# yanyan-li/PlanarSLAM

Hardware: AMD Instinct MI355X
Metric: RGB-D frames/sec (extract+match+pose-opt) @640x480; 1->8-GPU batch scaling (higher is better)
Workload: dtype u8/f64

## Files before the change

include/planar_abi.h:

```cpp
#ifndef PLANAR_ABI_H
#define PLANAR_ABI_H

#include <stdint.h>

#ifdef __cplusplus
extern "C" {
#endif

#define PLANAR_OK 0
#define PLANAR_EINVAL (-1)
#define PLANAR_ENOMEM (-2)
#define PLANAR_EDEVICE (-3)
#define PLANAR_ECAPACITY (-4)
#define PLANAR_ESTATE (-5)

typedef struct planar_ctx planar_ctx;

typedef struct planar_keypoint {
    float x, y;
    float size;
    float angle;
    float response;
    int32_t octave;
    int32_t class_id;
// ... 292 lines not shown
typedef struct planar_lsd planar_lsd;
int planar_lsd_create(planar_ctx* ctx, int width, int height, int max_batch, planar_lsd** out);
void planar_lsd_destroy(planar_lsd* lsd);
int planar_lsd_max_segments(void);
int planar_lsd_scaled_size(planar_lsd* lsd, int* w, int* h);
int planar_lsd_set_tie_order(planar_lsd* lsd, int tie_order);
int planar_lsd_set_top_only(planar_lsd* lsd, int enable);
int planar_lsd_extract(planar_lsd* lsd, const uint8_t* gray, int B, int pitch, int64_t frame_stride, int max_lines, planar_keyline* keylines,
                       uint8_t* ldesc, double* line_eq, int32_t* n_lines);
int planar_lsd_extract_dev(planar_lsd* lsd, const uint8_t* d_gray, int B, int pitch, int64_t frame_stride, int max_lines,
                           planar_keyline* d_keylines, uint8_t* d_ldesc, double* d_line_eq, int32_t* d_n_lines);
int planar_lsd_preprocess_dev(planar_lsd* lsd, const uint8_t* d_gray, int B, int pitch, int64_t frame_stride);
int planar_lsd_detect_dev(planar_lsd* lsd, int B, int max_lines, planar_keyline* d_keylines, uint8_t* d_ldesc, double* d_line_eq, int32_t* d_n_lines);
int planar_lsd_check(planar_lsd* lsd, int B);
int planar_lsd_read_stage(planar_lsd* lsd, int frame, int stage, void* out, int64_t out_bytes);
int planar_lsd_set_profiling(planar_lsd* lsd, int enable);
int planar_lsd_get_profile(planar_lsd* lsd, double* total_ms, int64_t* calls);
#ifdef PLANAR_TEST_HOOKS
int planar_debug_std_sort_desc(planar_ctx* ctx, float* keys, int32_t* perm, int n);
#endif

typedef struct planar_peac planar_peac;
int planar_peac_create(planar_ctx* ctx, int width, int height, int max_batch, planar_peac** out);
void planar_peac_destroy(planar_peac* peac);
int planar_peac_max_planes(void);
int planar_peac_segment(planar_peac* peac, const uint16_t* depth, int B, int pitch_px, int64_t frame_stride_px, float fx, float fy,
                        float cx, float cy, float depth_factor, int32_t* labels, double* planes, int32_t* n_planes);
int planar_peac_segment_dev(planar_peac* peac, const uint16_t* d_depth, int B, int pitch_px, int64_t frame_stride_px, float fx, float fy,
                            float cx, float cy, float depth_factor, int32_t* d_labels, double* d_planes, int32_t* d_n_planes);
int planar_peac_debug_layout(planar_peac* peac, int64_t* out );
int planar_peac_debug_read(planar_peac* peac, int frame, int64_t offset, int64_t bytes, void* out);
int planar_peac_check(planar_peac* peac, int B);
int planar_peac_set_variant(planar_peac* peac, int clustering, int wide_below);
int planar_peac_set_profiling(planar_peac* peac, int enable);
int planar_peac_get_profile(planar_peac* peac, double* total_ms, int64_t* calls);
int planar_peac_read_timing(planar_peac* peac, int B, int64_t* out);

typedef struct planar_comm planar_comm;
typedef struct planar_comm_id { char internal[128]; } planar_comm_id;
int planar_comm_unique_id(planar_comm_id* out);
int planar_comm_create(planar_ctx* ctx, const planar_comm_id* id, int nranks, int rank, planar_comm** out);
typedef int (*planar_allreduce_fn)(void* user, double* buf, size_t n, int op);
int planar_comm_create_hosted(planar_ctx* ctx, planar_allreduce_fn allreduce, void* user, int nranks, int rank, planar_comm** out);
void planar_comm_destroy(planar_comm* comm);

#define PLANAR_BA_MONO 0
#define PLANAR_BA_STEREO 1
#define PLANAR_BA_LINE 2
#define PLANAR_BA_PLANE 3
#define PLANAR_BA_VERTICAL 4
#define PLANAR_BA_PARALLEL 5

typedef struct planar_ba_problem {
    int32_t n_kf;
    const float* kf_Tcw;
    const uint8_t* kf_fixed;
    int32_t n_lm;
    const uint8_t* lm_type;
    const double* lm_init;
    int32_t n_edges;
    const int32_t* e_kf;
    const int32_t* e_lm;
    const uint8_t* e_type;
    const double* e_meas;
    const float* e_inv_sigma2;
} planar_ba_problem;
// ... 135 lines not shown
```

planarslam_amd/_lib.py:

```python
from __future__ import annotations

import ctypes as C
import os

import numpy as np

_HERE = os.path.dirname(os.path.abspath(__file__))
LIB_PATH = os.path.join(_HERE, "libplanar_hip.so")
if os.environ.get("PLANAR_HIP_LIB"):
    _ov = os.path.abspath(os.environ["PLANAR_HIP_LIB"])
    if os.path.dirname(_ov) != _HERE:
        raise ImportError(f"PLANAR_HIP_LIB={_ov}: a developer override must be a library inside {_HERE}")
    import warnings
    warnings.warn(f"planarslam_amd: loading the developer build {_ov} instead of libplanar_hip.so (PLANAR_HIP_LIB)")
    LIB_PATH = _ov

KP_DTYPE = np.dtype([("x", "<f4"), ("y", "<f4"), ("size", "<f4"), ("angle", "<f4"), ("response", "<f4"),
                     ("octave", "<i4"), ("class_id", "<i4")])


class PlanarError(RuntimeError):
    def __init__(self, code: int, msg: str):
        super().__init__(f"libplanar_hip error {code}: {msg}")
        self.code = code
# ... 134 lines not shown
    "planar_lsd_search_by_projection_dev": (C.c_int, [C.c_void_p, C.c_int, C.c_void_p, C.c_int, C.c_void_p, C.c_void_p, C.c_void_p, C.c_void_p, C.c_int] +
                                            [C.c_void_p] * 6 + [C.c_void_p, C.c_int, C.c_float, C.c_float, C.c_void_p, C.c_void_p]),
    "planar_plane_search_by_coefficients": (C.c_int, [C.c_void_p, C.c_int, C.c_void_p, C.c_int, C.c_void_p, C.c_void_p, C.c_int, C.c_void_p, C.c_int,
                                                      C.c_void_p, C.c_void_p, C.c_void_p, C.c_int, C.c_void_p, C.c_void_p] + [C.c_void_p] * 4),
    "planar_plane_search_by_coefficients_dev": (C.c_int, [C.c_void_p, C.c_int, C.c_void_p, C.c_int, C.c_void_p, C.c_void_p, C.c_int, C.c_void_p, C.c_int,
                                                          C.c_void_p, C.c_void_p, C.c_void_p, C.c_int, C.c_void_p, C.c_void_p] + [C.c_void_p] * 4),
    "planar_lsd_create": (C.c_int, [C.c_void_p, C.c_int, C.c_int, C.c_int, C.POINTER(C.c_void_p)]),
    "planar_lsd_destroy": (None, [C.c_void_p]),
    "planar_lsd_max_segments": (C.c_int, []),
    "planar_lsd_set_tie_order": (C.c_int, [C.c_void_p, C.c_int]),
    "planar_lsd_set_top_only": (C.c_int, [C.c_void_p, C.c_int]),
    "planar_undistort_keypoints": (C.c_int, [C.c_void_p, C.c_int, C.c_void_p, C.c_void_p, C.c_int] + [C.c_float] * 4 + [C.c_void_p, C.c_void_p]),
    "planar_undistort_keypoints_dev": (C.c_int, [C.c_void_p, C.c_int, C.c_void_p, C.c_void_p, C.c_int] + [C.c_float] * 4 + [C.c_void_p, C.c_void_p]),
    "planar_plane_clouds_sort_stats": (C.c_int, [C.c_void_p, C.c_int, C.c_void_p]),
    "planar_plane_clouds_set_profiling": (C.c_int, [C.c_void_p, C.c_int]),
    "planar_plane_clouds_get_profile": (C.c_int, [C.c_void_p, C.c_void_p, C.c_void_p]),
    "planar_lsd_set_profiling": (C.c_int, [C.c_void_p, C.c_int]),
    "planar_lsd_get_profile": (C.c_int, [C.c_void_p, C.c_void_p, C.c_void_p]),
    "planar_lsd_scaled_size": (C.c_int, [C.c_void_p, C.POINTER(C.c_int), C.POINTER(C.c_int)]),
    "planar_lsd_extract": (C.c_int, [C.c_void_p, C.c_void_p, C.c_int, C.c_int, C.c_int64, C.c_int, C.c_void_p, C.c_void_p, C.c_void_p, C.c_void_p]),
    "planar_lsd_extract_dev": (C.c_int, [C.c_void_p, C.c_void_p, C.c_int, C.c_int, C.c_int64, C.c_int, C.c_void_p, C.c_void_p, C.c_void_p, C.c_void_p]),
    "planar_lsd_preprocess_dev": (C.c_int, [C.c_void_p, C.c_void_p, C.c_int, C.c_int, C.c_int64]),
    "planar_lsd_detect_dev": (C.c_int, [C.c_void_p, C.c_int, C.c_int, C.c_void_p, C.c_void_p, C.c_void_p, C.c_void_p]),
    "planar_lsd_check": (C.c_int, [C.c_void_p, C.c_int]),
    "planar_lsd_read_stage": (C.c_int, [C.c_void_p, C.c_int, C.c_int, C.c_void_p, C.c_int64]),
    "planar_debug_std_sort_desc": (C.c_int, [C.c_void_p, C.c_void_p, C.c_void_p, C.c_int]),
    "planar_peac_create": (C.c_int, [C.c_void_p, C.c_int, C.c_int, C.c_int, C.POINTER(C.c_void_p)]),
    "planar_peac_destroy": (None, [C.c_void_p]),
    "planar_peac_max_planes": (C.c_int, []),
    "planar_peac_segment": (C.c_int, [C.c_void_p, C.c_void_p, C.c_int, C.c_int, C.c_int64, C.c_float, C.c_float, C.c_float, C.c_float, C.c_float, C.c_void_p, C.c_void_p, C.c_void_p]),
    "planar_peac_segment_dev": (C.c_int, [C.c_void_p, C.c_void_p, C.c_int, C.c_int, C.c_int64, C.c_float, C.c_float, C.c_float, C.c_float, C.c_float, C.c_void_p, C.c_void_p, C.c_void_p]),
    "planar_peac_check": (C.c_int, [C.c_void_p, C.c_int]),
    "planar_peac_set_variant": (C.c_int, [C.c_void_p, C.c_int, C.c_int]),
    "planar_track_manhattan_frame": (C.c_int, [C.c_void_p, C.c_int, C.c_void_p, C.c_void_p, C.c_void_p, C.c_int, C.c_void_p, C.c_void_p, C.c_int, C.c_void_p, C.c_void_p, C.c_void_p, C.c_void_p]),
    "planar_track_manhattan_frame_dev": (C.c_int, [C.c_void_p, C.c_int, C.c_void_p, C.c_void_p, C.c_void_p, C.c_int, C.c_void_p, C.c_void_p, C.c_int, C.c_void_p, C.c_void_p, C.c_void_p, C.c_void_p]),
    "planar_peac_read_timing": (C.c_int, [C.c_void_p, C.c_int, C.c_void_p]),
    "planar_reset_matches_dev": (C.c_int, [C.c_void_p, C.c_void_p, C.c_int64]),
    "planar_blocked_mask_dev": (C.c_int, [C.c_void_p, C.c_void_p, C.c_int64, C.c_void_p]),
    "planar_merge_matches_dev": (C.c_int, [C.c_void_p, C.c_void_p, C.c_void_p, C.c_int, C.c_int64, C.c_void_p]),
    "planar_manhattan_pose_dev": (C.c_int, [C.c_void_p, C.c_int, C.c_void_p, C.c_void_p, C.c_void_p, C.c_void_p]),
    "planar_keypoint_fields_dev": (C.c_int, [C.c_void_p, C.c_void_p, C.c_int64, C.c_void_p, C.c_void_p]),
    "planar_add_scalar_i32_dev": (C.c_int, [C.c_void_p, C.c_void_p, C.c_int64, C.c_int, C.c_void_p]),
    "planar_copy_rows_dev": (C.c_int, [C.c_void_p, C.c_void_p, C.c_int64, C.c_void_p, C.c_int64, C.c_int64, C.c_int64]),
    "planar_peac_debug_layout": (C.c_int, [C.c_void_p, C.c_void_p]),
    "planar_peac_debug_read": (C.c_int, [C.c_void_p, C.c_int, C.c_int64, C.c_int64, C.c_void_p]),
    "planar_comm_unique_id": (C.c_int, [C.c_void_p]),
    "planar_comm_create": (C.c_int, [C.c_void_p, C.c_void_p, C.c_int, C.c_int, C.POINTER(C.c_void_p)]),
    "planar_vocab_create": (C.c_int, [C.c_void_p, C.c_int, C.c_int, C.c_int, C.c_void_p, C.c_void_p, C.c_void_p, C.c_void_p, C.POINTER(C.c_void_p)]),
    "planar_vocab_destroy": (None, [C.c_void_p]),
    "planar_vocab_words": (C.c_int, [C.c_void_p]),
    "planar_bow_transform": (C.c_int, [C.c_void_p, C.c_void_p, C.c_void_p, C.c_int, C.c_int, C.c_int] + [C.c_void_p] * 6),
    "planar_bow_transform_dev": (C.c_int, [C.c_void_p, C.c_void_p, C.c_void_p, C.c_int, C.c_int, C.c_int] + [C.c_void_p] * 6),
    "planar_is_line_good": (C.c_int, [C.c_void_p, C.c_int, C.c_void_p, C.c_void_p, C.c_int, C.c_void_p, C.c_int, C.c_int, C.c_int, C.c_int64, C.c_float, C.c_float, C.c_float, C.c_float, C.c_float] + [C.c_void_p] * 8),
    "planar_is_line_good_dev": (C.c_int, [C.c_void_p, C.c_int, C.c_void_p, C.c_void_p, C.c_int, C.c_void_p, C.c_int, C.c_int, C.c_int, C.c_int64, C.c_float, C.c_float, C.c_float, C.c_float, C.c_float] + [C.c_void_p] * 8),
    "planar_normals_create": (C.c_int, [C.c_void_p, C.c_int, C.c_int, C.c_int, C.POINTER(C.c_void_p)]),
    "planar_normals_destroy": (None, [C.c_void_p]),
    "planar_normals_count": (C.c_int, [C.c_void_p]),
    "planar_normals_grid": (C.c_int, [C.c_void_p, C.POINTER(C.c_int), C.POINTER(C.c_int), C.POINTER(C.c_int), C.POINTER(C.c_int)]),
    "planar_normals_compute": (C.c_int, [C.c_void_p, C.c_void_p, C.c_int, C.c_int, C.c_int64, C.c_float, C.c_float, C.c_float, C.c_float, C.c_float, C.c_void_p, C.c_void_p]),
    "planar_normals_compute_dev": (C.c_int, [C.c_void_p, C.c_void_p, C.c_int, C.c_int, C.c_int64, C.c_float, C.c_float, C.c_float, C.c_float, C.c_float, C.c_void_p,
                                            C.c_void_p, C.c_int]),
    "planar_plane_clouds_create": (C.c_int, [C.c_void_p, C.c_int, C.c_int, C.c_int, C.c_int, C.POINTER(C.c_void_p)]),
    "planar_plane_clouds_destroy": (None, [C.c_void_p]),
    "planar_plane_clouds_set_timing": (C.c_int, [C.c_void_p, C.c_int]),
    "planar_plane_clouds_read_timing": (C.c_int, [C.c_void_p, C.c_int, C.c_void_p]),
    "planar_plane_clouds_stride": (C.c_int, [C.c_void_p, C.POINTER(C.c_int), C.POINTER(C.c_int)]),
# ... 100 lines not shown
```

planarslam_amd/csrc/common.h:

```cpp
#pragma once
#include <hip/hip_runtime.h>

#include <cstdarg>
#include <cstdint>
#include <cstdio>
#include <cstring>
#include <vector>

#include "../../include/planar_abi.h"

namespace planar {

void set_error(const char* fmt, ...);

#define PLANAR_HIP_CHECK(expr)                                                                        \
    do {                                                                                              \
        hipError_t _e = (expr);                                                                       \
        if (_e != hipSuccess) {                                                                       \
            ::planar::set_error("%s failed: %s (%s:%d)", #expr, hipGetErrorString(_e), __FILE__, __LINE__); \
            return (_e == hipErrorOutOfMemory) ? PLANAR_ENOMEM : PLANAR_EDEVICE;                      \
        }                                                                                             \
    } while (0)

#define PLANAR_REQUIRE(cond, code, msg)                  \
// ... 117 lines not shown
        for (int i = 0; i < slots; i++) total_ms[i] = 0;
        int64_t counted = 0;
        for (size_t c = 0; c < used; c++) {
            if (marked[c] != slots + 1) continue;
            for (int i = 0; i < slots; i++) {
                float ms = 0;
                PLANAR_HIP_CHECK(hipEventElapsedTime(&ms, ev[c * (slots + 1) + i], ev[c * (slots + 1) + i + 1]));
                total_ms[i] += ms;
            }
            counted++;
        }
        *calls = counted;
        reset();
        return PLANAR_OK;
    }
};

#ifdef __HIPCC__
__device__ __forceinline__ void xcd_frame_block(int per_frame, int B, int& frame, int& blk) {
    const int n = (int)blockIdx.x, group = 8 * per_frame, full = (B >> 3) * group;
    if (n < full) { const int g = n / group, r = n - g * group; frame = g * 8 + (r & 7); blk = r >> 3; }
    else { const int r = n - full; frame = (B & ~7) + r / per_frame; blk = r - (r / per_frame) * per_frame; }
}
#endif

}

struct planar_ctx {
    int device = 0;
    hipStream_t own_stream = nullptr;
    hipStream_t stream = nullptr;
    planar::DevBuf scratch;
    hipStream_t seq_stream = nullptr;
    hipEvent_t seq_fork = nullptr, seq_join = nullptr;
    hipStream_t seq_begin() {
        if (!seq_stream) return stream;
        hipError_t e = hipEventRecord(seq_fork, stream);
        if (e == hipSuccess) e = hipStreamWaitEvent(seq_stream, seq_fork, 0);
        if (e == hipSuccess) return seq_stream;
        planar::set_error("planar_ctx: the fork to the side stream failed (%s): launching on the context's stream", hipGetErrorString(e));
        return stream;
    }
    int seq_end(hipStream_t sq) {
        if (!seq_stream || sq != seq_stream) return PLANAR_OK;
        PLANAR_HIP_CHECK(hipEventRecord(seq_join, sq));
        PLANAR_HIP_CHECK(hipStreamWaitEvent(stream, seq_join, 0));
        return PLANAR_OK;
    }
    int ensure_scratch(size_t bytes) {
        if (scratch.bytes >= bytes) return PLANAR_OK;
        if (scratch.p) (void)hipStreamSynchronize(stream);
        return scratch.alloc(bytes);
    }
    void* host_scratch = nullptr;
    size_t host_scratch_bytes = 0;
    int ensure_host_scratch(size_t bytes) {
        if (host_scratch_bytes >= bytes) return PLANAR_OK;
        if (host_scratch) { (void)hipStreamSynchronize(stream); (void)hipHostFree(host_scratch); host_scratch = nullptr; host_scratch_bytes = 0; }
        const size_t want = planar::align_up(bytes + bytes / 4, (size_t)4096);
        hipError_t e = hipHostMalloc(&host_scratch, want, hipHostMallocDefault);
        if (e != hipSuccess) { (void)hipGetLastError(); host_scratch = nullptr; planar::set_error("hipHostMalloc(%zu) failed: %s", want, hipGetErrorString(e)); return PLANAR_EDEVICE; }
        host_scratch_bytes = want;
        return PLANAR_OK;
    }
};
```

planarslam_amd/csrc/ctx.hip:

```cpp
#include "common.h"

namespace planar {
static thread_local char g_err[512] = "";
void set_error(const char* fmt, ...) {
    va_list ap;
    va_start(ap, fmt);
    vsnprintf(g_err, sizeof(g_err), fmt, ap);
    va_end(ap);
}
}

extern "C" {

const char* planar_last_error(void) { return planar::g_err; }
int planar_abi_version(void) { return 200; }

int planar_ctx_create(planar_ctx** out, int device) {
    PLANAR_REQUIRE(out != nullptr, PLANAR_EINVAL, "out is null");
    *out = nullptr;
    int n = 0;
    PLANAR_HIP_CHECK(hipGetDeviceCount(&n));
    PLANAR_REQUIRE(device >= 0 && device < n, PLANAR_EDEVICE, "no such HIP device");
    PLANAR_HIP_CHECK(hipSetDevice(device));
    planar_ctx* c = new (std::nothrow) planar_ctx();
    PLANAR_REQUIRE(c != nullptr, PLANAR_ENOMEM, "host allocation failed");
    c->device = device;
    hipError_t e = hipStreamCreateWithFlags(&c->own_stream, hipStreamNonBlocking);
    if (e != hipSuccess) { delete c; planar::set_error("hipStreamCreate failed: %s", hipGetErrorString(e)); return PLANAR_EDEVICE; }
    c->stream = c->own_stream;
    *out = c;
    return PLANAR_OK;
}

void planar_ctx_destroy(planar_ctx* ctx) {
    if (!ctx) return;
    if (ctx->seq_fork) (void)hipEventDestroy(ctx->seq_fork);
    if (ctx->seq_join) (void)hipEventDestroy(ctx->seq_join);
    if (ctx->host_scratch) (void)hipHostFree(ctx->host_scratch);
    if (ctx->own_stream) (void)hipStreamDestroy(ctx->own_stream);
    delete ctx;
}

int planar_ctx_set_stream(planar_ctx* ctx, void* s) {
    PLANAR_REQUIRE(ctx != nullptr, PLANAR_EINVAL, "ctx is null");
    ctx->stream = s ? (hipStream_t)s : ctx->own_stream;
    return PLANAR_OK;
}

int planar_cu_stream_create(int device, const uint32_t* cu_mask, int n_words, void** out_stream) {
    PLANAR_REQUIRE(out_stream && cu_mask && n_words >= 1 && n_words <= 32, PLANAR_EINVAL, "bad argument");
    *out_stream = nullptr;
    bool any = false;
    for (int i = 0; i < n_words; i++) any = any || cu_mask[i] != 0u;
    PLANAR_REQUIRE(any, PLANAR_EINVAL, "empty CU mask");
    PLANAR_HIP_CHECK(hipSetDevice(device));
    hipStream_t s = nullptr;
    PLANAR_HIP_CHECK(hipExtStreamCreateWithCUMask(&s, (uint32_t)n_words, cu_mask));
    *out_stream = (void*)s;
    return PLANAR_OK;
}

void planar_cu_stream_destroy(void* stream) { if (stream) (void)hipStreamDestroy((hipStream_t)stream); }

int planar_ctx_set_seq_stream(planar_ctx* ctx, void* s) {
    PLANAR_REQUIRE(ctx != nullptr, PLANAR_EINVAL, "ctx is null");
    PLANAR_HIP_CHECK(hipSetDevice(ctx->device));
    if (s && !ctx->seq_fork) {
        PLANAR_HIP_CHECK(hipEventCreateWithFlags(&ctx->seq_fork, hipEventDisableTiming));
        PLANAR_HIP_CHECK(hipEventCreateWithFlags(&ctx->seq_join, hipEventDisableTiming));
    }
    ctx->seq_stream = (hipStream_t)s;
    return PLANAR_OK;
}

void* planar_ctx_get_stream(planar_ctx* ctx) { return ctx ? (void*)ctx->stream : nullptr; }

int planar_ctx_sync(planar_ctx* ctx) {
    PLANAR_REQUIRE(ctx != nullptr, PLANAR_EINVAL, "ctx is null");
    PLANAR_HIP_CHECK(hipStreamSynchronize(ctx->stream));
    return PLANAR_OK;
}

}
```

planarslam_amd/csrc/peac.hip:

```cpp
#include "common.h"

#include "peac_common.h"

namespace planar {
namespace peac {

constexpr int NT_REFINE = 256;
constexpr int NT_REFINE_WIDE = 1024;

struct Lds {
    float* h_key; u16* h_id; u16* pool; u16* nb_off; u16* nb_cnt; u16* dsp; u16* dss; u16* rid; unsigned* nouse; signed char* blk;
};

__device__ __forceinline__ int lds_find(u16* parent, int x) {
    int r = x, guard = 0;
    while (parent[r] != r && ++guard < 8192) r = parent[r];
    guard = 0;
    while (parent[x] != r && ++guard < 8192) { const int nx = parent[x]; parent[x] = (u16)r; x = nx; }
    return r;
}
template <int NT, int FJ>
__device__ __forceinline__ void refine_frame(const Layout& L, const Intr& K, const Consts& C, const uint16_t* __restrict__ depth, int pitch_px,
                                             int64_t frame_stride_px, uint8_t* __restrict__ ws, int32_t* __restrict__ labels,
                                             int64_t label_stride, double* __restrict__ planes, int32_t* __restrict__ n_planes,
                                             int32_t* __restrict__ status, long long* __restrict__ timing, const int frame) {
    const int tid = threadIdx.x, lane = tid & 63, wave = tid >> 6;
    uint8_t* F = ws + (size_t)frame * L.frame_bytes;
    double* g_stats = (double*)(F + L.off_stats);
    double* g_geo = (double*)(F + L.off_geo);
    int* g_N = (int*)(F + L.off_N);
    signed char* member = (signed char*)(F + L.off_member);
    float* distMap = (float*)(F + L.off_dist);
    unsigned* queue = (unsigned*)(F + L.off_queue);
// ... 718 lines not shown
                                                  int64_t frame_stride_px, uint8_t* __restrict__ ws, int32_t* __restrict__ labels,
                                                  int64_t label_stride, double* __restrict__ planes, int32_t* __restrict__ n_planes,
                                                  int32_t* __restrict__ status, long long* __restrict__ timing) {
    refine_frame<NT_REFINE_WIDE, 4>(L, K, C, depth, pitch_px, frame_stride_px, ws, labels, label_stride, planes, n_planes, status, timing, (int)blockIdx.x);
}

__global__ void peac_order(const long long* __restrict__ timing, int B, int* __restrict__ order) {
    const int i = blockIdx.x * blockDim.x + threadIdx.x;
    if (i >= B) return;
    const long long ci = timing[(size_t)i * TSLOTS + 3];
    int rank = 0;
    for (int j = 0; j < B; j++) {
        const long long cj = timing[(size_t)j * TSLOTS + 3];
        rank += (cj > ci || (cj == ci && j < i)) ? 1 : 0;
    }
    order[rank] = i;
}

}
}

#include "peac_ahc2.h"

using namespace planar;

struct planar_peac {
    planar_ctx* ctx = nullptr;
    int W = 0, H = 0, max_batch = 0;
    peac::Layout L{};
    peac::Consts C{};
    int smem2 = 0, smem3 = 0, smem_refine = 0;
    int wide_below = 64;
    bool exact_only = false;
    DevBuf d_ws, d_status, d_timing, d_next, d_order;
    int order_B = 0;
    DevBuf d_depth, d_labels, d_planes, d_nplanes;
    LaunchProfile prof{4};
};

extern "C" {

int planar_peac_create(planar_ctx* ctx, int width, int height, int max_batch, planar_peac** out) {
    PLANAR_REQUIRE(ctx && out, PLANAR_EINVAL, "null argument");
    *out = nullptr;
    PLANAR_REQUIRE(width >= 2 * peac::WIN && height >= 2 * peac::WIN && width <= 4096 && height <= 4096, PLANAR_EINVAL, "image size out of range");
    PLANAR_REQUIRE(max_batch >= 1, PLANAR_EINVAL, "max_batch must be >= 1");
    PLANAR_HIP_CHECK(hipSetDevice(ctx->device));
    planar_peac* o = new (std::nothrow) planar_peac();
    PLANAR_REQUIRE(o != nullptr, PLANAR_ENOMEM, "host allocation failed");
    o->ctx = ctx; o->W = width; o->H = height; o->max_batch = max_batch;
    o->L = peac::make_layout(width, height);
    o->C = peac::make_consts();
    const peac::Layout& L = o->L;
    o->smem2 = peac::ahc2_smem_bytes(L);
    o->smem3 = peac::ahc3_smem_bytes(L);
    o->smem_refine = (int)((L.NB + 15) / 16 * 16);
    if (L.pool_cap > 65535 || L.NB2 > 65535 || o->smem2 > 160 * 1024 - 2048 || o->smem3 > o->smem2) {
        delete o;
        set_error("planar_peac_create: %dx%d = %d blocks of 10x10 pixels: the clustering kernel's LDS-resident queue holds about 10 900 (1280x720 fits, 1920x1080 does not)", width, height, L.NB);
        return PLANAR_EINVAL;
    }
    if (o->smem2 > 48 * 1024) {
        hipError_t e = hipSuccess;
        if (o->smem3 > 48 * 1024) e = hipFuncSetAttribute((const void*)peac::peac_ahc3, hipFuncAttributeMaxDynamicSharedMemorySize, o->smem3);
        if (e == hipSuccess) e = hipFuncSetAttribute((const void*)peac::peac_ahc2, hipFuncAttributeMaxDynamicSharedMemorySize, o->smem2);
        if (e != hipSuccess) { (void)hipGetLastError(); delete o; set_error("planar_peac_create: %d bytes of LDS per workgroup are not available: %s", o->smem2, hipGetErrorString(e)); return PLANAR_EINVAL; }
    }
    int rc;
    if ((rc = o->d_ws.alloc((size_t)max_batch * L.frame_bytes)) || (rc = o->d_status.alloc((size_t)max_batch * 4)) ||
        (rc = o->d_timing.alloc((size_t)max_batch * peac::TSLOTS * 8)) || (rc = o->d_next.alloc(256)) || (rc = o->d_order.alloc((size_t)max_batch * 4))) { delete o; return rc; }
    *out = o;
    return PLANAR_OK;
}

void planar_peac_destroy(planar_peac* p) { delete p; }
int planar_peac_set_variant(planar_peac* p, int clustering, int wide_below) {
    PLANAR_REQUIRE(p && clustering >= 0 && clustering <= 1, PLANAR_EINVAL, "bad argument");
    p->exact_only = clustering == 1;
    if (wide_below >= 0) p->wide_below = wide_below;
    return PLANAR_OK;
}
int planar_peac_max_planes(void) { return peac::MAX_PLANES; }

int planar_peac_segment_dev(planar_peac* p, const uint16_t* d_depth, int B, int pitch_px, int64_t frame_stride_px, float fx, float fy,
                            float cx, float cy, float depth_factor, int32_t* d_labels, double* d_planes, int32_t* d_n_planes) {
    PLANAR_REQUIRE(p && d_depth && d_labels && d_planes && d_n_planes, PLANAR_EINVAL, "null argument");
    PLANAR_REQUIRE(B >= 1 && B <= p->max_batch, PLANAR_EINVAL, "B must be in [1, max_batch]");
    PLANAR_REQUIRE(pitch_px >= p->W && frame_stride_px >= (int64_t)pitch_px * p->H, PLANAR_EINVAL, "pitch/frame_stride too small");
    hipStream_t st = p->ctx->stream;
    const peac::Intr K{fx, fy, cx, cy, depth_factor};
    int rc = p->prof.begin();
    if (rc) return rc;
    auto mark = [&]() { p->prof.mark(st); };
    PLANAR_HIP_CHECK(hipMemsetAsync(p->d_next.p, 0, 4, st));
    mark();
    hipLaunchKernelGGL(peac::peac_blocks, dim3((p->L.NB + 63) / 64, B), dim3(64), 0, st, p->L, K, d_depth, pitch_px, frame_stride_px, p->d_ws.as<uint8_t>());
    mark();
    {
        hipStream_t sq = p->ctx->seq_begin();
        if (!p->exact_only) {
            hipLaunchKernelGGL(peac::peac_ahc3, dim3(B), dim3(64), p->smem3, sq, p->L, p->C, p->d_ws.as<uint8_t>(), p->d_status.as<int32_t>(),
                               p->d_timing.as<long long>(), p->d_next.as<int>(), p->order_B == B ? p->d_order.as<int>() : nullptr, 0);
            hipLaunchKernelGGL(peac::peac_ahc2, dim3(B), dim3(64), p->smem2, sq, p->L, p->C, p->d_ws.as<uint8_t>(), p->d_status.as<int32_t>(),
                               p->d_timing.as<long long>(), p->d_next.as<int>(), nullptr, 1);
        } else
            hipLaunchKernelGGL(peac::peac_ahc2, dim3(B), dim3(64), p->smem2, sq, p->L, p->C, p->d_ws.as<uint8_t>(), p->d_status.as<int32_t>(),
                               p->d_timing.as<long long>(), p->d_next.as<int>(), p->order_B == B ? p->d_order.as<int>() : nullptr, 0);
        if ((rc = p->ctx->seq_end(sq))) return rc;
    }
    mark();
    hipLaunchKernelGGL(peac::peac_order, dim3((B + 255) / 256), dim3(256), 0, st, p->d_timing.as<long long>(), B, p->d_order.as<int>());
    mark();
    if (B <= p->wide_below)
        hipLaunchKernelGGL(peac::peac_refine_wide, dim3(B), dim3(peac::NT_REFINE_WIDE), p->smem_refine, st, p->L, K, p->C, d_depth, pitch_px, frame_stride_px,
                           p->d_ws.as<uint8_t>(), d_labels, (int64_t)p->W * p->H, d_planes, d_n_planes, p->d_status.as<int32_t>(), p->d_timing.as<long long>());
    else
        hipLaunchKernelGGL(peac::peac_refine, dim3(B), dim3(peac::NT_REFINE), p->smem_refine, st, p->L, K, p->C, d_depth, pitch_px, frame_stride_px,
                           p->d_ws.as<uint8_t>(), d_labels, (int64_t)p->W * p->H, d_planes, d_n_planes, p->d_status.as<int32_t>(), p->d_timing.as<long long>());
    mark();
    p->order_B = B;
    PLANAR_HIP_CHECK(hipGetLastError());
    return PLANAR_OK;
}

int planar_peac_set_profiling(planar_peac* p, int enable) {
    PLANAR_REQUIRE(p != nullptr, PLANAR_EINVAL, "peac is null");
    PLANAR_HIP_CHECK(hipStreamSynchronize(p->ctx->stream));
    p->prof.on = enable != 0;
    p->prof.reset();
    return PLANAR_OK;
}
int planar_peac_get_profile(planar_peac* p, double* total_ms , int64_t* calls) {
    PLANAR_REQUIRE(p && total_ms && calls, PLANAR_EINVAL, "null argument");
    PLANAR_HIP_CHECK(hipStreamSynchronize(p->ctx->stream));
    return p->prof.sum(total_ms, calls);
}

int planar_peac_read_timing(planar_peac* p, int B, int64_t* out) {
    PLANAR_REQUIRE(p && out && B >= 1 && B <= p->max_batch, PLANAR_EINVAL, "bad argument");
    PLANAR_HIP_CHECK(hipStreamSynchronize(p->ctx->stream));
    PLANAR_HIP_CHECK(hipMemcpy(out, p->d_timing.p, (size_t)B * peac::TSLOTS * 8, hipMemcpyDeviceToHost));
    return PLANAR_OK;
}

// ... 53 lines not shown
```

planarslam_amd/csrc/peac_ahc2.h:

```cpp
#pragma once
#include "peac_common.h"
#include "wave_ops.h"

namespace planar {
namespace peac {

constexpr unsigned TOMB = 0xFFFFu;
#define WFENCE() do { __builtin_amdgcn_fence(__ATOMIC_SEQ_CST, "wavefront"); __builtin_amdgcn_wave_barrier(); } while (0)
#define GFENCE() __threadfence_block()

__device__ __forceinline__ void stats_compute_u(const double s[9], int N, Geo& g) {
    const double sc = 1.0 / N;
    g.center[0] = s[0] * sc; g.center[1] = s[1] * sc; g.center[2] = s[2] * sc;
    const double k00 = s[3] - s[0] * s[0] * sc, k01 = s[6] - s[0] * s[1] * sc, k02 = s[8] - s[0] * s[2] * sc;
    const double k11 = s[4] - s[1] * s[1] * sc, k12 = s[7] - s[1] * s[2] * sc, k22 = s[5] - s[2] * s[2] * sc;
    double ev[3], v[3];
    eig33u(k00, k01, k11, k02, k12, k22, ev, v);
    const bool keep = v[0] * g.center[0] + v[1] * g.center[1] + v[2] * g.center[2] <= 0;
    g.normal[0] = keep ? v[0] : -v[0]; g.normal[1] = keep ? v[1] : -v[1]; g.normal[2] = keep ? v[2] : -v[2];
    g.mse = ev[0] * sc;
}

__host__ __device__ static inline size_t al8(size_t v) { return (v + 7) & ~(size_t)7; }
static inline int ahc2_smem_bytes(const Layout& L) {
// ... 928 lines not shown
    WFENCE();
    mark();
    {
        unsigned* o_nouse = (unsigned*)(F + L.off_h_nouse); unsigned* o_cval = (unsigned*)(F + L.off_h_cval);
        const int W32o = (NB2 + 31) / 32;
        for (int b0 = 0; b0 < NB2; b0 += 64) {
            const int id = b0 + lane;
            bool dead;
            if constexpr (FAST) {
                if (id < NB) dead = mp[id] != id || (rec(id)[2] >> 16) != (unsigned)id;
                else dead = id < n_nodes;
            } else dead = id < NB2 && mp[id] != id;
            const u64 dm = __ballot(dead);
            if (lane == 0) { o_nouse[b0 >> 5] = (unsigned)dm; if ((b0 >> 5) + 1 < W32o) o_nouse[(b0 >> 5) + 1] = (unsigned)(dm >> 32); }
        }
        if constexpr (FAST) {
            GFENCE();
            for (int id = lane; id < NB; id += 64) {
                const unsigned c = rec(id)[2] >> 16;
                if (mp[id] == id && c >= (unsigned)NB) atomicAnd(&o_nouse[c >> 5], ~(1u << (c & 31)));
            }
        }
        for (int t = lane; t < (NB2 + 31) / 32; t += 64) o_cval[t] = 0;
        for (int t = lane; t < MAX_PLANES; t += 64) g_hand[4 + t] = t < n_ext ? (FAST ? (int)(rec(s_ext[t])[2] >> 16) : s_ext[t]) : 0;
        if (lane == 0) {
            g_hand[0] = n_ext; g_hand[1] = err; g_hand[2] = n_nodes;
            status[frame] = err;
            if (timing) {
                for (int t = 0; t < 4; t++) timing[(size_t)frame * TSLOTS + t] = t < nph ? tphase[t] - tphase[0] : 0;
                timing[(size_t)frame * TSLOTS + 9] = n_nodes;
                timing[(size_t)frame * TSLOTS + 7] = ((long long)dbg_phases << 40) | ((long long)dbg_nodes << 20) | dbg_hits;
                timing[(size_t)frame * TSLOTS + 10] = dbg_big;
                timing[(size_t)frame * TSLOTS + 11] = dbg_bigsolves;
                for (int t = 0; t < 24; t++) timing[(size_t)frame * TSLOTS + 16 + t] = cyc[t];
            }
        }
    }
    return wave_uni(err);
}

__global__ __launch_bounds__(64, 2) void peac_ahc3(Layout L, Consts C, uint8_t* __restrict__ ws, int32_t* __restrict__ status,
                                                   long long* __restrict__ timing, int* __restrict__ next_frame, const int* __restrict__ order, int retry_inline) {
    __shared__ int s_frame;
    __shared__ AhcShared s_sh;
#if defined(PLANAR_AHC_PRIO) && !defined(PLANAR_WAVE_EMUL)
    __builtin_amdgcn_s_setprio(PLANAR_AHC_PRIO);
#endif
    if (threadIdx.x == 0) { const int k = atomicAdd(next_frame, 1); s_frame = order ? order[k] : k; }
    __syncthreads();
    const int st = ahc_frame<true>(L, C, ws, status, timing, s_frame, s_sh);
    if (st == ST_RETRY && retry_inline) {
        __syncthreads();
        ahc_frame<false>(L, C, ws, status, timing, s_frame, s_sh);
        if (timing && threadIdx.x == 0) timing[(size_t)s_frame * TSLOTS + 12] = 1;
    }
}
__global__ __launch_bounds__(64) void peac_ahc2(Layout L, Consts C, uint8_t* __restrict__ ws, int32_t* __restrict__ status,
                                                long long* __restrict__ timing, int* __restrict__ next_frame, const int* __restrict__ order, int only_retry) {
    __shared__ int s_frame;
    __shared__ AhcShared s_sh;
    if (threadIdx.x == 0) {
        if (only_retry) s_frame = status[blockIdx.x] == ST_RETRY ? (int)blockIdx.x : -1;
        else { const int k = atomicAdd(next_frame, 1); s_frame = order ? order[k] : k; }
    }
    __syncthreads();
    if (s_frame < 0) return;
    ahc_frame<false>(L, C, ws, status, timing, s_frame, s_sh);
}

}
}
```

planarslam_amd/planes.py:

```python
from __future__ import annotations

import ctypes as C

import numpy as np

from ._lib import Context, PlanarError, check, lib


class PlaneDetection:
    def __init__(self, width: int = 640, height: int = 480, max_batch: int = 1, ctx: Context | None = None):
        self.L = lib()
        self.ctx = ctx or Context(0)
        self.width, self.height, self.max_batch = width, height, max_batch
        h = C.c_void_p()
        check(self.L.planar_peac_create(self.ctx.h, width, height, max_batch, C.byref(h)))
        self.h = h
        self.max_planes = self.L.planar_peac_max_planes()

    def close(self):
        if getattr(self, "h", None):
            self.L.planar_peac_destroy(self.h)
            self.h = None

    def __del__(self):
        try:
            self.close()
        except Exception:
            pass

    def run(self, depth: np.ndarray, K=(535.4, 539.2, 320.1, 247.6), depth_factor: float = 1.0 / 5000.0):
        if depth.dtype != np.uint16:
            raise TypeError("depth image must be CV_16U (uint16)")
        single = depth.ndim == 2
        d = np.ascontiguousarray(depth[None] if single else depth)
        B, H, W = d.shape
        if (W, H) != (self.width, self.height):
            raise ValueError(f"detector was created for {self.width}x{self.height}, got {W}x{H}")
        labels = np.zeros((B, H, W), np.int32)
        planes = np.zeros((B, self.max_planes, 8), np.float64)
        n = np.zeros(B, np.int32)
        check(self.L.planar_peac_segment(self.h, d.ctypes.data, B, W, W * H, K[0], K[1], K[2], K[3], np.float32(depth_factor),
                                         labels.ctypes.data, planes.ctypes.data, n.ctypes.data))
        res = [(planes[b, :n[b]].copy(), labels[b]) for b in range(B)]
        return res[0] if single else res

    def segment_dev(self, d_depth, d_labels, d_planes, d_n, B, K=(535.4, 539.2, 320.1, 247.6), depth_factor=1.0 / 5000.0):
        check(self.L.planar_peac_segment_dev(self.h, d_depth, B, self.width, self.width * self.height, K[0], K[1], K[2], K[3],
                                             np.float32(depth_factor), d_labels, d_planes, d_n))


class SurfaceNormals:

    def __init__(self, width: int = 640, height: int = 480, max_batch: int = 1, ctx: Context | None = None):
        self.L = lib()
        self.ctx = ctx or Context(0)
        self.width, self.height, self.max_batch = width, height, max_batch
        h = C.c_void_p()
        check(self.L.planar_normals_create(self.ctx.h, width, height, max_batch, C.byref(h)))
        self.h = h
        self.count = check(self.L.planar_normals_count(self.h))

# ... 171 lines not shown
```

Before: 12670.

## Make PEAC clustering kernels persistent and size grids by occupancy and CU mask

The ahc3 and ahc2 clustering kernels become persistent loops. Each workgroup keeps pulling frames from an atomic counter, and the grid is sized from occupancy times the CU count, using the seq stream's CU mask when one is set. Frames that need a retry go onto a device-side list, so the retry pass runs a small fixed grid over only those frames instead of launching B workgroups that mostly exit. The order kernel moves onto the seq stream, and a cap on workgroups is exposed. This is meant to cut launch and scheduling overhead and to balance frames of uneven cost, at the price of more atomics and kernarg reloads inside the loop.

```diff
diff --git a/include/planar_abi.h b/include/planar_abi.h
--- a/include/planar_abi.h
+++ b/include/planar_abi.h
@@ -348,6 +348,7 @@
 int planar_peac_debug_read(planar_peac* peac, int frame, int64_t offset, int64_t bytes, void* out);
 int planar_peac_check(planar_peac* peac, int B);
 int planar_peac_set_variant(planar_peac* peac, int clustering, int wide_below);
+int planar_peac_set_max_workgroups(planar_peac* peac, int n);
 int planar_peac_set_profiling(planar_peac* peac, int enable);
 int planar_peac_get_profile(planar_peac* peac, double* total_ms, int64_t* calls);
 int planar_peac_read_timing(planar_peac* peac, int B, int64_t* out);
diff --git a/planarslam_amd/_lib.py b/planarslam_amd/_lib.py
--- a/planarslam_amd/_lib.py
+++ b/planarslam_amd/_lib.py
@@ -190,6 +190,7 @@
     "planar_peac_segment_dev": (C.c_int, [C.c_void_p, C.c_void_p, C.c_int, C.c_int, C.c_int64, C.c_float, C.c_float, C.c_float, C.c_float, C.c_float, C.c_void_p, C.c_void_p, C.c_void_p]),
     "planar_peac_check": (C.c_int, [C.c_void_p, C.c_int]),
     "planar_peac_set_variant": (C.c_int, [C.c_void_p, C.c_int, C.c_int]),
+    "planar_peac_set_max_workgroups": (C.c_int, [C.c_void_p, C.c_int]),
     "planar_track_manhattan_frame": (C.c_int, [C.c_void_p, C.c_int, C.c_void_p, C.c_void_p, C.c_void_p, C.c_int, C.c_void_p, C.c_void_p, C.c_int, C.c_void_p, C.c_void_p, C.c_void_p, C.c_void_p]),
     "planar_track_manhattan_frame_dev": (C.c_int, [C.c_void_p, C.c_int, C.c_void_p, C.c_void_p, C.c_void_p, C.c_int, C.c_void_p, C.c_void_p, C.c_int, C.c_void_p, C.c_void_p, C.c_void_p, C.c_void_p]),
     "planar_peac_read_timing": (C.c_int, [C.c_void_p, C.c_int, C.c_void_p]),
diff --git a/planarslam_amd/csrc/common.h b/planarslam_amd/csrc/common.h
--- a/planarslam_amd/csrc/common.h
+++ b/planarslam_amd/csrc/common.h
@@ -173,6 +173,7 @@
     hipStream_t stream = nullptr;
     planar::DevBuf scratch;
     hipStream_t seq_stream = nullptr;
+    int seq_cus = 0;
     hipEvent_t seq_fork = nullptr, seq_join = nullptr;
     hipStream_t seq_begin() {
         if (!seq_stream) return stream;
diff --git a/planarslam_amd/csrc/ctx.hip b/planarslam_amd/csrc/ctx.hip
--- a/planarslam_amd/csrc/ctx.hip
+++ b/planarslam_amd/csrc/ctx.hip
@@ -13,7 +13,7 @@
 extern "C" {
 
 const char* planar_last_error(void) { return planar::g_err; }
-int planar_abi_version(void) { return 200; }
+int planar_abi_version(void) { return 201; }
 
 int planar_ctx_create(planar_ctx** out, int device) {
     PLANAR_REQUIRE(out != nullptr, PLANAR_EINVAL, "out is null");
@@ -70,6 +70,12 @@
         PLANAR_HIP_CHECK(hipEventCreateWithFlags(&ctx->seq_join, hipEventDisableTiming));
     }
     ctx->seq_stream = (hipStream_t)s;
+    ctx->seq_cus = 0;
+    if (s) {
+        uint32_t mask[32] = {0};
+        if (hipExtStreamGetCUMask((hipStream_t)s, 32, mask) == hipSuccess) { for (uint32_t w : mask) ctx->seq_cus += __builtin_popcount(w); }
+        else (void)hipGetLastError();
+    }
     return PLANAR_OK;
 }
 
diff --git a/planarslam_amd/csrc/peac.hip b/planarslam_amd/csrc/peac.hip
--- a/planarslam_amd/csrc/peac.hip
+++ b/planarslam_amd/csrc/peac.hip
@@ -1,4 +1,6 @@
 #include "common.h"
+
+#include <algorithm>
 
 #include "peac_common.h"
 
@@ -783,6 +785,7 @@
     int smem2 = 0, smem3 = 0, smem_refine = 0;
     int wide_below = 64;
     bool exact_only = false;
+    int occ3 = 0, occ2 = 0, dev_cus = 0, max_wg = 0;
     DevBuf d_ws, d_status, d_timing, d_next, d_order;
     int order_B = 0;
     DevBuf d_depth, d_labels, d_planes, d_nplanes;
@@ -817,9 +820,19 @@
         if (e == hipSuccess) e = hipFuncSetAttribute((const void*)peac::peac_ahc2, hipFuncAttributeMaxDynamicSharedMemorySize, o->smem2);
         if (e != hipSuccess) { (void)hipGetLastError(); delete o; set_error("planar_peac_create: %d bytes of LDS per workgroup are not available: %s", o->smem2, hipGetErrorString(e)); return PLANAR_EINVAL; }
     }
+    {
+        hipError_t e = hipOccupancyMaxActiveBlocksPerMultiprocessor(&o->occ3, (const void*)peac::peac_ahc3, 64, (size_t)o->smem3);
+        if (e == hipSuccess) e = hipOccupancyMaxActiveBlocksPerMultiprocessor(&o->occ2, (const void*)peac::peac_ahc2, 64, (size_t)o->smem2);
+        if (e == hipSuccess) e = hipDeviceGetAttribute(&o->dev_cus, hipDeviceAttributeMultiprocessorCount, ctx->device);
+        if (e != hipSuccess || o->occ3 < 1 || o->occ2 < 1 || o->dev_cus < 1) {
+            (void)hipGetLastError(); delete o;
+            set_error("planar_peac_create: the clustering kernels' residency is not available: %s", hipGetErrorString(e));
+            return PLANAR_EDEVICE;
+        }
+    }
     int rc;
     if ((rc = o->d_ws.alloc((size_t)max_batch * L.frame_bytes)) || (rc = o->d_status.alloc((size_t)max_batch * 4)) ||
-        (rc = o->d_timing.alloc((size_t)max_batch * peac::TSLOTS * 8)) || (rc = o->d_next.alloc(256)) || (rc = o->d_order.alloc((size_t)max_batch * 4))) { delete o; return rc; }
+        (rc = o->d_timing.alloc((size_t)max_batch * peac::TSLOTS * 8)) || (rc = o->d_next.alloc(256 + (size_t)max_batch * 4)) || (rc = o->d_order.alloc((size_t)max_batch * 4))) { delete o; return rc; }
     *out = o;
     return PLANAR_OK;
 }
@@ -829,6 +842,11 @@
     PLANAR_REQUIRE(p && clustering >= 0 && clustering <= 1, PLANAR_EINVAL, "bad argument");
     p->exact_only = clustering == 1;
     if (wide_below >= 0) p->wide_below = wide_below;
+    return PLANAR_OK;
+}
+int planar_peac_set_max_workgroups(planar_peac* p, int n) {
+    PLANAR_REQUIRE(p && n >= 0, PLANAR_EINVAL, "bad argument");
+    p->max_wg = n;
     return PLANAR_OK;
 }
 int planar_peac_max_planes(void) { return peac::MAX_PLANES; }
@@ -843,24 +861,29 @@
     int rc = p->prof.begin();
     if (rc) return rc;
     auto mark = [&]() { p->prof.mark(st); };
-    PLANAR_HIP_CHECK(hipMemsetAsync(p->d_next.p, 0, 4, st));
+    PLANAR_HIP_CHECK(hipMemsetAsync(p->d_next.p, 0, (1 + peac::RETRY_LIST) * 4, st));
     mark();
     hipLaunchKernelGGL(peac::peac_blocks, dim3((p->L.NB + 63) / 64, B), dim3(64), 0, st, p->L, K, d_depth, pitch_px, frame_stride_px, p->d_ws.as<uint8_t>());
     mark();
     {
         hipStream_t sq = p->ctx->seq_begin();
+        const int cus = (sq != st && sq == p->ctx->seq_stream && p->ctx->seq_cus > 0) ? std::min(p->ctx->seq_cus, p->dev_cus) : p->dev_cus;
+        auto grid = [&](int per_cu) { const int g = std::min(B, per_cu * cus); return dim3((unsigned)(p->max_wg > 0 ? std::min(g, p->max_wg) : g)); };
+        int* d_next = p->d_next.as<int>();
+        const int* order = p->order_B == B ? p->d_order.as<int>() : nullptr;
         if (!p->exact_only) {
-            hipLaunchKernelGGL(peac::peac_ahc3, dim3(B), dim3(64), p->smem3, sq, p->L, p->C, p->d_ws.as<uint8_t>(), p->d_status.as<int32_t>(),
-                               p->d_timing.as<long long>(), p->d_next.as<int>(), p->order_B == B ? p->d_order.as<int>() : nullptr, 0);
-            hipLaunchKernelGGL(peac::peac_ahc2, dim3(B), dim3(64), p->smem2, sq, p->L, p->C, p->d_ws.as<uint8_t>(), p->d_status.as<int32_t>(),
-                               p->d_timing.as<long long>(), p->d_next.as<int>(), nullptr, 1);
+            hipLaunchKernelGGL(peac::peac_ahc3, grid(p->occ3), dim3(64), p->smem3, sq, p->L, p->C, p->d_ws.as<uint8_t>(), p->d_status.as<int32_t>(),
+                               p->d_timing.as<long long>(), d_next, order, 0, B, d_next + 1);
+            const int g2 = std::min(B, peac::RETRY_GRID);
+            hipLaunchKernelGGL(peac::peac_ahc2, dim3((unsigned)(p->max_wg > 0 ? std::min(g2, p->max_wg) : g2)), dim3(64), p->smem2, sq, p->L, p->C, p->d_ws.as<uint8_t>(),
+                               p->d_status.as<int32_t>(), p->d_timing.as<long long>(), d_next, (const int*)nullptr, 1, B, d_next + 1);
         } else
-            hipLaunchKernelGGL(peac::peac_ahc2, dim3(B), dim3(64), p->smem2, sq, p->L, p->C, p->d_ws.as<uint8_t>(), p->d_status.as<int32_t>(),
-                               p->d_timing.as<long long>(), p->d_next.as<int>(), p->order_B == B ? p->d_order.as<int>() : nullptr, 0);
+            hipLaunchKernelGGL(peac::peac_ahc2, grid(p->occ2), dim3(64), p->smem2, sq, p->L, p->C, p->d_ws.as<uint8_t>(), p->d_status.as<int32_t>(),
+                               p->d_timing.as<long long>(), d_next, order, 0, B, (int*)nullptr);
+        hipLaunchKernelGGL(peac::peac_order, dim3((B + 255) / 256), dim3(256), 0, sq, p->d_timing.as<long long>(), B, p->d_order.as<int>());
         if ((rc = p->ctx->seq_end(sq))) return rc;
     }
     mark();
-    hipLaunchKernelGGL(peac::peac_order, dim3((B + 255) / 256), dim3(256), 0, st, p->d_timing.as<long long>(), B, p->d_order.as<int>());
     mark();
     if (B <= p->wide_below)
         hipLaunchKernelGGL(peac::peac_refine_wide, dim3(B), dim3(peac::NT_REFINE_WIDE), p->smem_refine, st, p->L, K, p->C, d_depth, pitch_px, frame_stride_px,
diff --git a/planarslam_amd/csrc/peac_ahc2.h b/planarslam_amd/csrc/peac_ahc2.h
--- a/planarslam_amd/csrc/peac_ahc2.h
+++ b/planarslam_amd/csrc/peac_ahc2.h
@@ -984,6 +984,7 @@
                 timing[(size_t)frame * TSLOTS + 7] = ((long long)dbg_phases << 40) | ((long long)dbg_nodes << 20) | dbg_hits;
                 timing[(size_t)frame * TSLOTS + 10] = dbg_big;
                 timing[(size_t)frame * TSLOTS + 11] = dbg_bigsolves;
+                timing[(size_t)frame * TSLOTS + 12] = 0;
                 for (int t = 0; t < 24; t++) timing[(size_t)frame * TSLOTS + 16 + t] = cyc[t];
             }
         }
@@ -991,33 +992,73 @@
     return wave_uni(err);
 }
 
+constexpr int RETRY_COUNT = 0, RETRY_TAKEN = 1, RETRY_LIST = 3;
+constexpr int RETRY_GRID = 64;
+
 __global__ __launch_bounds__(64, 2) void peac_ahc3(Layout L, Consts C, uint8_t* __restrict__ ws, int32_t* __restrict__ status,
-                                                   long long* __restrict__ timing, int* __restrict__ next_frame, const int* __restrict__ order, int retry_inline) {
+                                                   long long* __restrict__ timing, int* __restrict__ next_frame, const int* __restrict__ order, int retry_inline,
+                                                   int B = 1, int* __restrict__ retry = nullptr) {
     __shared__ int s_frame;
     __shared__ AhcShared s_sh;
 #if defined(PLANAR_AHC_PRIO) && !defined(PLANAR_WAVE_EMUL)
     __builtin_amdgcn_s_setprio(PLANAR_AHC_PRIO);
 #endif
-    if (threadIdx.x == 0) { const int k = atomicAdd(next_frame, 1); s_frame = order ? order[k] : k; }
-    __syncthreads();
-    const int st = ahc_frame<true>(L, C, ws, status, timing, s_frame, s_sh);
-    if (st == ST_RETRY && retry_inline) {
+#ifdef PLANAR_WAVE_EMUL
+    for (;;) {
+        if (threadIdx.x == 0) { const int k = atomicAdd(next_frame, 1); s_frame = k < B ? (order ? order[k] : k) : -1; }
         __syncthreads();
-        ahc_frame<false>(L, C, ws, status, timing, s_frame, s_sh);
-        if (timing && threadIdx.x == 0) timing[(size_t)s_frame * TSLOTS + 12] = 1;
-    }
+        const int frame = wave_uni(s_frame);
+        if (frame < 0) break;
+        const int st = ahc_frame<true>(L, C, ws, status, timing, frame, s_sh);
+        if (st == ST_RETRY) {
+            if (retry_inline) {
+                __syncthreads();
+                ahc_frame<false>(L, C, ws, status, timing, frame, s_sh);
+                if (timing && threadIdx.x == 0) timing[(size_t)frame * TSLOTS + 12] = 1;
+            } else if (retry && threadIdx.x == 0) retry[RETRY_LIST + atomicAdd(&retry[RETRY_COUNT], 1)] = frame;
+        }
+        __syncthreads();
+    }
+#elif defined(__HIP_DEVICE_COMPILE__)
+    struct Args { Layout L; Consts C; uint8_t* ws; int32_t* status; long long* timing; int* next_frame; const int* order; int retry_inline; int B; int* retry; };
+    for (;;) {
+        auto kp = __builtin_amdgcn_kernarg_segment_ptr();
+        asm volatile("" : "+s"(kp));
+        const __attribute__((address_space(4))) Args& A = *(const __attribute__((address_space(4))) Args*)kp;
+        if (threadIdx.x == 0) { const int k = atomicAdd(A.next_frame, 1); s_frame = k < A.B ? (A.order ? A.order[k] : k) : -1; }
+        __syncthreads();
+        const int frame = wave_uni(s_frame);
+        if (frame < 0) break;
+        const Layout Lf = A.L; const Consts Cf = A.C;
+        const int st = ahc_frame<true>(Lf, Cf, A.ws, A.status, A.timing, frame, s_sh);
+        if (st == ST_RETRY && A.retry && threadIdx.x == 0) A.retry[RETRY_LIST + atomicAdd(&A.retry[RETRY_COUNT], 1)] = frame;
+        __syncthreads();
+    }
+#else
+    (void)s_frame; (void)s_sh;
+#endif
 }
 __global__ __launch_bounds__(64) void peac_ahc2(Layout L, Consts C, uint8_t* __restrict__ ws, int32_t* __restrict__ status,
-                                                long long* __restrict__ timing, int* __restrict__ next_frame, const int* __restrict__ order, int only_retry) {
+                                                long long* __restrict__ timing, int* __restrict__ next_frame, const int* __restrict__ order, int only_retry,
+                                                int B = 1, int* __restrict__ retry = nullptr) {
     __shared__ int s_frame;
     __shared__ AhcShared s_sh;
-    if (threadIdx.x == 0) {
-        if (only_retry) s_frame = status[blockIdx.x] == ST_RETRY ? (int)blockIdx.x : -1;
-        else { const int k = atomicAdd(next_frame, 1); s_frame = order ? order[k] : k; }
-    }
-    __syncthreads();
-    if (s_frame < 0) return;
-    ahc_frame<false>(L, C, ws, status, timing, s_frame, s_sh);
+    for (;;) {
+        if (threadIdx.x == 0) {
+            int f = -1;
+            if (only_retry) {
+                const int n = retry ? min(retry[RETRY_COUNT], B) : 0;
+                if (n > 0) { const int k = atomicAdd(&retry[RETRY_TAKEN], 1); if (k < n) f = retry[RETRY_LIST + k]; }
+            } else { const int k = atomicAdd(next_frame, 1); if (k < B) f = order ? order[k] : k; }
+            s_frame = f;
+        }
+        __syncthreads();
+        const int frame = wave_uni(s_frame);
+        if (frame < 0 || frame >= B) break;
+        ahc_frame<false>(L, C, ws, status, timing, frame, s_sh);
+        if (only_retry && timing && threadIdx.x == 0) timing[(size_t)frame * TSLOTS + 12] = 1;
+        __syncthreads();
+    }
 }
 
 }
diff --git a/planarslam_amd/planes.py b/planarslam_amd/planes.py
--- a/planarslam_amd/planes.py
+++ b/planarslam_amd/planes.py
@@ -27,6 +27,9 @@
             self.close()
         except Exception:
             pass
+
+    def set_max_workgroups(self, n: int):
+        check(self.L.planar_peac_set_max_workgroups(self.h, int(n)))
 
     def run(self, depth: np.ndarray, K=(535.4, 539.2, 320.1, 247.6), depth_factor: float = 1.0 / 5000.0):
         if depth.dtype != np.uint16:
```

Result: no change. 12690 (median of 3 runs) (+0.2%).
